# hahnyuan/PTQ4ViT

Hardware: AMD Instinct MI355X
Metric: calibration throughput (wrapped modules calibrated per second), ViT-B/224 W8A8, 32 calibration images (higher is better)
Workload: dtype int8

## Files before the change

ptq4vit_amd/csrc/p4v_api.hip:

```cpp
#include <hip/hip_runtime.h>

#include <algorithm>
#include <atomic>
#include <climits>
#include <cstdarg>
#include <cstdio>
#include <condition_variable>
#include <cstring>
#include <deque>
#include <functional>
#include <thread>
#include <mutex>
#include <string>
#include <unordered_map>
#include <type_traits>
#include <vector>

#include "../../include/ptq4vit_hip.h"
#include "../../include/ptq4vit_hip_debug.h"
#include "p4v_kernels.h"

using namespace p4v;

namespace {
// ... 499 lines not shown
    return p.mode == PACK_SYM && !p.conv && !(p.blk_mode == 1 && p.blk_div2) && p.lo >= -128 && p.hi <= 127 && p.lo <= p.hi &&
           (p.crange ? live_max == 1 : p.C == 1) && (p.c_inner != 3 || (p.Rp % 64 == 0 && p.Kp % 64 == 0));
}
std::atomic<int> g_pack_general{0};
template <typename T> int launch_pack(Ctx& c, const PackParams& p_, int live_max = -1) {
    if (c.dry) return 0;
    PackParams p = p_;
    if (p.crange && live_max == 0) return 0;
    p.qbias = (sizeof(T) == 1 && p.mode == PACK_SYM && p.lo == -128 && p.hi == 127 && tune(TUNE_B1_PATH) != 11) ? cvt_bias(c) : 0.0f;
    const long total = (long)p.Z * p.Rp * (p.Kp / 16);
    if (total >= (1L << 31)) return fail(P4V_ERR_UNSUPPORTED, "operand plane too large for k_pack (%ld 16-element runs)", total);
    const int groups = cdiv((p.crange && live_max > 0) ? std::min(p.C, live_max) : p.C, PACK_CG);
    const long cap = !p.crange ? 256L * 64 : live_max > 0 ? std::max(256L * 12, 256L * 64 / groups) : 256L * 12;
    const int blocks = (int)std::min<long>(cdiv(total, 256), cap);
    if (p.mode == PACK_TWIN_I8) {
        if (sizeof(T) != 1 || p.C != 1 || p.c_inner != 0 || !p.scales || p.conv || p.zdiv > 0)
            return fail(P4V_ERR_UNSUPPORTED, "merged twin plane: one fixed row-major int8 plane only");
        return enqueue(c, KERN(PackParams, k_pack_twin), dim3(blocks), dim3(256), 0, p);
    }
    const bool single = sizeof(T) == 1 && pack1_ok(p, live_max) && !g_pack_general.load(std::memory_order_relaxed);
    if (tune(TUNE_PRINT) > 1) fprintf(stderr, "[p4v] %s stage %d: Z %d Rp %d Kp %d C %d crange %d done %d live_max %d layout %d grid %d x %d\n", single ? "k_pack1" : "k_pack", g_stage, p.Z, p.Rp, p.Kp, p.C, p.crange != nullptr, p.done != nullptr, live_max, p.c_inner, blocks, single ? 1 : groups);
    if (single) return enqueue(c, KERN(PackParams, k_pack1), dim3(blocks), dim3(256), 0, p);
    return enqueue(c, KERN_T(PackParams, k_pack, T), dim3(blocks, groups), dim3(256), 0, p);
}

inline int lockstep(const Ctx& c, int kind) {
    if (!c.grp) return 1;
    const int seen = (kind >= 0 && kind < 16) ? c.grp->last_par[kind] : 0;
    return std::max(1, seen > 0 ? seen : c.par);
}
inline int cu_slots(const Ctx& c, int slots, int kind) { return std::max(8, slots / lockstep(c, kind)); }
#define P4V_EPI4(epi, X)                                   \
    switch (epi) {                                         \
        case EPI_SQ_W: { constexpr int E = EPI_SQ_W; X; }  \
        case EPI_SQ: { constexpr int E = EPI_SQ; X; }      \
        case EPI_ABS: { constexpr int E = EPI_ABS; X; }    \
        default: { constexpr int E = EPI_W_SQ; X; }        \
    }

template <typename T, bool TWIN> int launch_sweep_epi(Ctx& c, const SweepParams& p, int epi, int cgroups, const StatInfo* si) {
    const size_t lds = 2 * (TWIN ? 3 : 2) * SW_TILE_BYTES;
    dim3 grid(p.mtiles * p.ntiles, p.Z, cgroups), block(512);
    switch (epi) {
        case EPI_SQ_W: return enqueue(c, KERN_T(SweepParams, k_sweep, T, TWIN, EPI_SQ_W), grid, block, lds, p, si);
        case EPI_SQ: return enqueue(c, KERN_T(SweepParams, k_sweep, T, TWIN, EPI_SQ), grid, block, lds, p, si);
        case EPI_ABS: return enqueue(c, KERN_T(SweepParams, k_sweep, T, TWIN, EPI_ABS), grid, block, lds, p, si);
        case EPI_W_SQ: return enqueue(c, KERN_T(SweepParams, k_sweep, T, TWIN, EPI_W_SQ), grid, block, lds, p, si);
        case EPI_STORE: return enqueue(c, KERN1_T(SweepParams, k_sweep, T, TWIN, EPI_STORE), grid, block, lds, p, si);
        case EPI_FWD: return enqueue(c, KERN1_T(SweepParams, k_sweep, T, TWIN, EPI_FWD), grid, block, lds, p, si);
        default: return enqueue(c, KERN1_T(SweepParams, k_sweep, T, TWIN, EPI_COS), grid, block, lds, p, si);
    }
}

template <bool TWIN> int launch_sweep2g_epi(Ctx& c, const SweepParams& p, int epi, int cgroups, const StatInfo* si) {
    const int per = 2 * cdiv(p.c1 - p.c0, 2 * cgroups);
    const size_t lds = (size_t)SW2_NS * (TWIN ? 4 : 3) * SW2_TILE + (size_t)per * 8 * sizeof(float) * (TWIN ? 3 : 2);
    dim3 grid(p.mtiles * p.ntiles, p.Z, cgroups), block(512);
    P4V_EPI4(epi, return enqueue(c, KERN_T(SweepParams, k_sweep2g, TWIN, E), grid, block, lds, p, si))
}

template <bool TWIN> int launch_sweep2_epi(Ctx& c, const SweepParams& p, int epi, int cgroups, const StatInfo* si) {
    const int per = cdiv(p.c1 - p.c0, cgroups);
    const size_t lds = (size_t)SW2_NS * (TWIN ? 3 : 2) * SW2_TILE + (size_t)per * 8 * sizeof(float) * (TWIN ? 3 : 2);
    dim3 grid(p.mtiles * p.ntiles, p.Z, cgroups), block(512);
    switch (epi) {
        case EPI_SQ_W: return enqueue(c, KERN_T(SweepParams, k_sweep2, TWIN, EPI_SQ_W), grid, block, lds, p, si);
        case EPI_SQ: return enqueue(c, KERN_T(SweepParams, k_sweep2, TWIN, EPI_SQ), grid, block, lds, p, si);
        case EPI_ABS: return enqueue(c, KERN_T(SweepParams, k_sweep2, TWIN, EPI_ABS), grid, block, lds, p, si);
        case EPI_FWD: return enqueue(c, KERN1_T(SweepParams, k_sweep2, TWIN, EPI_FWD), grid, block, lds, p, si);
        case EPI_STORE:
            if constexpr (TWIN) return enqueue(c, KERN1_T(SweepParams, k_sweep2, TWIN, EPI_STORE), grid, block, lds, p, si);
            else return enqueue(c, KERN_T(SweepParams, k_sweep2, TWIN, EPI_STORE), grid, block, lds, p, si);
        case EPI_COS: return enqueue(c, KERN_T(SweepParams, k_sweep2, TWIN, EPI_COS), grid, block, lds, p, si);
        default: return enqueue(c, KERN_T(SweepParams, k_sweep2, TWIN, EPI_W_SQ), grid, block, lds, p, si);
    }
}

#ifdef P4V_TRACE
unsigned long long* g_trace = nullptr;
int trace_attach(Sweep3Params& p) {
    if (!g_trace) HIPCHK(hipMalloc(&g_trace, sizeof(unsigned long long) * 16 * 65536));
    p.trace = g_trace;
    return 0;
}
int trace_dump(Ctx& c, dim3 grid, int ktiles) {
    if (!getenv("P4V_TRACE_FILE")) return 0;
    const size_t n = (size_t)grid.x * grid.z * 16;
    HIPCHK(hipStreamSynchronize(c.st));
    std::vector<unsigned long long> h(n);
    HIPCHK(hipMemcpy(h.data(), g_trace, n * 8, hipMemcpyDeviceToHost));
    FILE* f = fopen(getenv("P4V_TRACE_FILE"), "ab");
    unsigned long long hdr[4] = {0xABCDull, grid.x, grid.z, (unsigned long long)ktiles};
    fwrite(hdr, 8, 4, f); fwrite(h.data(), 8, n, f); fclose(f);
    return 0;
}
#endif

inline StatInfo stat_info(int kind, double macs, double alg, int gx, int gz, double bytes) {
    return StatInfo{kind, macs * g_exec_frac, alg * g_exec_frac, g_stage, gx, gz, bytes};
}

enum SweepKind { SK_BOUND, SK_SWEEP6, SK_SWEEP5, SK_SWEEP7, SK_SWEEP7_TWIN, SK_SWEEP7_MERGED, SK_SWEEP9, SK_SWEEP8, SK_SWEEP2G, SK_SWEEP2,
                 SK_GENERIC_I8, SK_GENERIC_F32, SK_COUNT };
constexpr int SWEEP_RECORD_KIND[SK_COUNT] = {12, 2, 5, 3, 4, 4, 6, 7, 8, 9, 0, 1};
inline bool sweep_stationary(SweepKind k) { return k == SK_SWEEP6 || k == SK_SWEEP5; }
inline bool sweep_large_k(SweepKind k) { return k == SK_SWEEP7 || k == SK_SWEEP7_TWIN || k == SK_SWEEP7_MERGED; }

int launch_sweep5(Ctx& c, const Sweep3Params& p, int epi, int cgroups) {
    if (c.dry) return 0;
    const int per = 2 * cdiv(p.c1 - p.c0, 2 * cgroups);
    const size_t lds = (size_t)p.ktiles * SW2_TILE + (size_t)SW5_NP * 2 * SW2_TILE + (size_t)per * 8 * sizeof(float) * 2 + 256;
    dim3 grid(p.stiles * p.ttiles, 1, cgroups), block(512);
#ifdef P4V_TRACE
    CHK(trace_attach(const_cast<Sweep3Params&>(p)));
#endif
    const StatInfo si = stat_info(SWEEP_RECORD_KIND[SK_SWEEP5], (double)p.stiles * 128 * (double)p.ttiles * 128 * (double)p.ldk * (p.c1 - p.c0), g_alg_macs_cand * (p.c1 - p.c0),
                                  (int)grid.x, (int)grid.z, g_alg_bytes);
    const StatInfo* sp = &si;
    P4V_EPI4(epi, CHK(enqueue(c, KERN_T(Sweep3Params, k_sweep5, E), grid, block, lds, p, sp)); break)
#ifdef P4V_TRACE
    CHK(trace_dump(c, grid, p.ktiles));
#endif
    return 0;
}

template <int KT>
int launch_sweep6_kt(Ctx& c, const Sweep3Params& p, int epi, dim3 grid, size_t lds, const StatInfo* si) {
    if (epi == EPI_COS) return enqueue(c, KERN_T(Sweep3Params, k_sweep6, EPI_COS, KT, 2), grid, dim3(256), lds, p, si);
    if (epi == EPI_COS_T) return enqueue(c, KERN_T(Sweep3Params, k_sweep6, EPI_COS_T, KT, 2), grid, dim3(256), lds, p, si);
    P4V_EPI4(epi, return enqueue(c, KERN_T(Sweep3Params, k_sweep6, E, KT, 2), grid, dim3(256), lds, p, si))
}

bool sweep6_supported(int ktiles) { return ktiles == 3 || ktiles == 4 || ktiles == 6 || ktiles == 8 || ktiles == 12; }

int launch_sweep6_part(Ctx& c, const Sweep3Params& p, int epi, int cgroups);

int launch_sweep6(Ctx& c, const Sweep3Params& p, int epi, int cgroups, int nc_model = 0) {
    if (c.dry) return 0;
    const int tiles = p.ntile > 0 ? p.ntile : p.stiles * p.ttiles, base = p.ntile > 0 ? p.tile0 : 0;
    const int nc = nc_model > 0 ? nc_model : p.c1 - p.c0;
    const int full = tiles / 256 * 256, rem = tiles - full;
    const double P = tune(TUNE_P6) > 0 ? 0.1 * tune(TUNE_P6) : 20.0, t_c = 0.196 * p.ktiles;
    auto waves = [](long wgs) { return (double)((wgs + 255) / 256); };
    int q_best = 0;
    if (rem > 0 && full > 0 && lockstep(c, 2) <= 1) {
        double best = waves((long)tiles * cgroups) * (P + cdiv(nc, cgroups) * t_c) * 0.97;
        for (int q = 1; q <= std::min(nc, 12); ++q) {
            const double t = waves(full) * (P + nc * t_c) + waves((long)rem * q) * (P + cdiv(nc, q) * t_c);
            if (t < best) { best = t; q_best = q; }
        }
    }
    if (tune(TUNE_PRINT) > 0) fprintf(stderr, "[p4v] sweep6 tiles %d: full %d rem %d -> q %d (uniform cg %d)\n", tiles, full, rem, q_best, cgroups);
    if (q_best > 0) {
        Sweep3Params a = p, b = p;
        a.tile0 = base; a.ntile = full;
        b.tile0 = base + full; b.ntile = rem;
        CHK(launch_sweep6_part(c, a, epi, 1));
// ... 21 lines not shown
    int r;
    switch (p.ktiles) {
        case 12: r = launch_sweep6_kt<12>(c, p, epi, grid, lds, sp); break;
        case 8: r = launch_sweep6_kt<8>(c, p, epi, grid, lds, sp); break;
        case 6: r = launch_sweep6_kt<6>(c, p, epi, grid, lds, sp); break;
        case 4: r = launch_sweep6_kt<4>(c, p, epi, grid, lds, sp); break;
        default: r = launch_sweep6_kt<3>(c, p, epi, grid, lds, sp); break;
    }
    if (r) return r;
#ifdef P4V_TRACE
    CHK(trace_dump(c, grid, p.ktiles));
#endif
    return 0;
}

template <bool ROWS_FIXED> int launch_sweep9_epi(Ctx& c, const SweepParams& p, int epi, int cgroups, const StatInfo* si) {
    const int per = cdiv(p.c1 - p.c0, cgroups);
    const size_t lds = (size_t)SW9_NS * SW9_STAGE + (size_t)per * SW9_NW * sizeof(float) * 2;
    dim3 grid(p.halves, p.Z, cgroups), block(SW9_NW * 64);
    P4V_EPI4(epi, return enqueue(c, KERN_T(SweepParams, k_sweep9, ROWS_FIXED, E), grid, block, lds, p, si))
}

template <bool ROWS_FIXED> int launch_sweep8_epi(Ctx& c, const SweepParams& p, int epi, int cgroups, const StatInfo* si) {
    const int per = cdiv(p.c1 - p.c0, cgroups);
    const size_t lds = (size_t)SW8_NS * SW2_TILE + (size_t)per * 8 * sizeof(float) * 2;
    dim3 grid(p.mtiles * p.ntiles, p.Z, cgroups), block(512);
    P4V_EPI4(epi, return enqueue(c, KERN_T(SweepParams, k_sweep8, ROWS_FIXED, E, false), grid, block, lds, p, si))
}

template <int TWIN> int launch_sweep7_epi(Ctx& c, const Sweep7Params& p, int epi, dim3 grid, size_t lds, const StatInfo* si) {
    if constexpr (TWIN == 0) { if (epi == EPI_COS) return enqueue(c, KERN_T(Sweep7Params, k_sweep7, 0, EPI_COS), grid, dim3(512), lds, p, si); }
    if (epi == EPI_COS) return fail(P4V_ERR_UNSUPPORTED, "k_sweep7: the cosine epilogue has no twin instance");
    P4V_EPI4(epi, return enqueue(c, KERN_T(Sweep7Params, k_sweep7, TWIN, E), grid, dim3(512), lds, p, si))
}

int launch_sweep7(Ctx& c, const Sweep7Params& p, int twin, int epi, int cgroups) {
    if (c.dry) return 0;
    const int nc = p.c1 - p.c0;
    const int per_max = (int)((160 * 1024 - SW7_NS * SW7_STAGE - 256) / 192);
    cgroups = std::max(cgroups, cdiv(nc, per_max));
    const int per = cdiv(nc, cgroups);
    const size_t lds = (size_t)SW7_NS * SW7_STAGE + (size_t)per * 192 + 256;
    Sweep7Params q = p;
    q.cgroups = cgroups;
    dim3 grid(p.rtiles * p.ctiles * cgroups, 1, 1);
    const StatInfo si = stat_info(SWEEP_RECORD_KIND[twin ? SK_SWEEP7_TWIN : SK_SWEEP7], (double)p.rtiles * 256 * (double)p.ctiles * 256 * (double)p.ldk * nc, g_alg_macs_cand * nc,
                                  (int)grid.x, (int)grid.z, g_alg_bytes);
    const StatInfo* sp = &si;
    return twin == 2 ? launch_sweep7_epi<2>(c, q, epi, grid, lds, sp) : twin ? launch_sweep7_epi<1>(c, q, epi, grid, lds, sp) : launch_sweep7_epi<0>(c, q, epi, grid, lds, sp);
}

int launch_sweep(Ctx& c, const SweepParams& p, SweepKind kind, bool twin, int epi, int cgroups) {
    if (c.dry) return 0;
    const double kelems = (double)p.ldk / (kind == SK_GENERIC_F32 ? 4 : 1);
    const int tiles = p.mtiles * p.ntiles;
    auto record = [&](int gx) {
        return stat_info(SWEEP_RECORD_KIND[kind], (double)p.mtiles * SW_BM * (double)p.ntiles * SW_BN * kelems * p.Z * (p.c1 - p.c0) * (twin ? 2 : 1),
                         g_alg_macs_cand * (p.c1 - p.c0), gx, cgroups, g_alg_bytes);
    };
    switch (kind) {
        case SK_BOUND: {
            const bool prev = b1_previous();
            const StatInfo si = record(tiles * (prev ? 2 : 1));
            const dim3 grid(tiles * (prev ? 2 : 1)), block(256);
            if (prev) P4V_EPI4(epi, return enqueue(c, KERN_T(SweepParams, k_bound, E, 1), grid, block, 0, p, &si))
            P4V_EPI4(epi, return enqueue(c, KERN_T(SweepParams, k_bound, E, 2), grid, block, 0, p, &si))
        }
        case SK_SWEEP9: {
            const StatInfo si = record(p.halves);
            return p.a_cs == 0 ? launch_sweep9_epi<true>(c, p, epi, cgroups, &si) : launch_sweep9_epi<false>(c, p, epi, cgroups, &si);
        }
        case SK_SWEEP8: {
            const StatInfo si = record(tiles);
            return p.a_cs == 0 ? launch_sweep8_epi<true>(c, p, epi, cgroups, &si) : launch_sweep8_epi<false>(c, p, epi, cgroups, &si);
        }
        case SK_SWEEP2G: {
            const StatInfo si = record(tiles);
            return twin ? launch_sweep2g_epi<true>(c, p, epi, cgroups, &si) : launch_sweep2g_epi<false>(c, p, epi, cgroups, &si);
        }
        case SK_SWEEP2: {
            const StatInfo si = record(tiles);
            return twin ? launch_sweep2_epi<true>(c, p, epi, cgroups, &si) : launch_sweep2_epi<false>(c, p, epi, cgroups, &si);
        }
        case SK_GENERIC_I8: {
            const StatInfo si = record(tiles);
            return twin ? launch_sweep_epi<int8_t, true>(c, p, epi, cgroups, &si) : launch_sweep_epi<int8_t, false>(c, p, epi, cgroups, &si);
        }
        case SK_GENERIC_F32: {
            const StatInfo si = record(tiles);
            return twin ? launch_sweep_epi<float, true>(c, p, epi, cgroups, &si) : launch_sweep_epi<float, false>(c, p, epi, cgroups, &si);
        }
        default: return fail(P4V_ERR_INVALID, "launch_sweep: family %d has a launcher of its own", (int)kind);
    }
}

int launch_finish(Ctx& c, const FinishParams& p) {
    return enqueue(c, KERN(FinishParams, k_finish), dim3(p.C, p.nj), dim3(256), 0, p);
}

int launch_finish_cos(Ctx& c, const FinishCosParams& p) {
    const int gy = p.j_mode == 3 ? cdiv(p.S, 256) : p.nj;
    return enqueue(c, KERN(FinishCosParams, k_finish_cos), dim3(p.C, gy), dim3(p.j_mode == 3 ? 256 : 1024), 0, p);
}

int launch_select(Ctx& c, const SelectParams& p_) {
    if (c.dry) return 0;
    SelectParams p = p_;
    attach_mirror(p);
    return enqueue(c, KERN(SelectParams, k_select), dim3(p.nj), dim3(128), 0, p);
}

struct PlaneCache {
    char* buf = nullptr;
    bool assigned = false, valid = false;
    unsigned char* done = nullptr;
};
struct SliceCache {
    bool assigned = false;
    int k = 0;
    int k_eff = 0;
    int* idx = nullptr; float* mass = nullptr;
    float* Os = nullptr; float* Gs = nullptr; float* Rs = nullptr;
    const void* idx_src = nullptr; int idx_wt = -1;
    const void* o_src = nullptr; const void* g_src = nullptr; const void* r_src = nullptr;
    float* frac = nullptr;
    PlaneCache aplane;
    bool loose = false;
    float frac_host = 1.0f;
};
typedef PlaneCache EpiCache;

struct Operand {
    PackParams pk;
    bool expanded;
    bool present;
};

struct SegPlan {
    SegTable seg; unsigned char ablk[SEG_MAX], bblk[SEG_MAX]; int Kseg;
    int batch, H, M, K, N;
    int nVA, nHA, nVB, nHB, crA, ccA, crB, ccB;
    const float* A; long a_st[4]; const float* B; long b_st[4];
    int Aq, Bq; bool sos;
// ... 204 lines not shown
    long part_cs;
    long p_zs, p_cs; int NpP;
    int s3_groups, cos6_Sp;
    int h9;
    long fin_zs; int fin_ld, fin_rows, fin_cols, fin_jdiv;
};

int sweep9_halves(const Pass& ps, int ktiles) {
    const int epi = ps.epi;
    if (ktiles != 1 || ps.twin || ps.row.expanded == ps.col.expanded || epi == EPI_STORE || epi == EPI_FWD || epi == EPI_COS) return 0;
    if (ps.sb_mode == 1 && ps.s_cs > 1) return 0;
    if (ps.bias_axis != 0 || (g_variant & 524288)) return 0;
    if ((ps.row.expanded ? ps.Mrows : ps.Ncols) > 256) return 0;
    const long nb = (long)cdiv(ps.Mrows, 16) * cdiv(ps.Ncols, 16);
    const int halves = (int)cdiv(nb, (long)SW9_NW * SW9_NB);
    if (halves > 32 / SW9_NW) return 0;
    const double waste = (double)rup(ps.Mrows, 128) * rup(ps.Ncols, 128) / ((double)rup(ps.Mrows, 16) * rup(ps.Ncols, 16));
    return (waste >= 1.4 || (g_variant & 1048576)) ? halves : 0;
}
bool sweep8_ok(const Pass& ps, int ktiles) {
    return ktiles == 1 && !ps.twin && ps.row.expanded != ps.col.expanded && ps.epi != EPI_STORE && ps.epi != EPI_FWD && ps.epi != EPI_COS &&
           !(g_variant & 65536);
}
bool sweep2g_ok(const Pass& ps, int ktiles) {
    return ps.col.expanded && !ps.row.expanded && ktiles >= 16 && ps.o_bs == 0 && ps.o_nbs == 0 && ps.epi != EPI_COS;
}

int plan_sweep(const Ctx& c, const Pass& ps, SweepPlan& pl) {
    pl = SweepPlan{};
    const int esz = pl.esz = ps.i8 ? 1 : 4;
    const int Kp = pl.Kp = (int)rup(ps.K, 64 / esz);
    const int ktiles = Kp * esz / SW_BKB;
    const long K64 = rup(ps.K, 64);
    const bool cosm = ps.epi == EPI_COS, i8v2 = ps.i8 && !g_force_v1;
    const bool one_expanded = ps.row.expanded != ps.col.expanded, plain_out = ps.o_bs == 0 && ps.o_nbs == 0;
    const bool scale32 = ps.sb_mode != 1 || ps.s_cs == 1 || ps.sb_div % 32 == 0;
    const bool score32 = ps.j_mode == 0 || (ps.j_mode == 1 && (ps.nj == 1 || ps.j_div % 32 == 0));
    const bool blocks64 = (ps.s_cs == 1 || ps.sb_div % 64 == 0) && (ps.j_mode == 0 || (ps.j_mode == 1 && (ps.nj == 1 || ps.j_div % 64 == 0)));
    const bool bound = ps.bound_kernel && i8v2 && !ps.twin && ps.Z == 1 && !ps.store_out && !cosm && plain_out && ps.bias_axis == 0 &&
                       (ps.sb_mode == 0 || ps.sb_mode == 1) && score32 && scale32 && (ps.eq_n == 1 || ps.crange);
    const bool stat_ok = !bound && !ps.store_out && i8v2 && !ps.twin && (!cosm || ps.cos6) && !(g_variant & 4) && ps.Z == 1 &&
                         ps.sb_mode == 1 && blocks64 && one_expanded && K64 <= 768 && plain_out;
    const bool regs6 = stat_ok && sweep6_supported(ktiles);
    if (ps.cos6 && !regs6) return fail(P4V_ERR_UNSUPPORTED, "cosine pass planned for k_sweep6 does not qualify for it");
    const bool big7 = !bound && !stat_ok && !ps.store_out && i8v2 && (!cosm || ps.cos7) && !(g_variant & 32768) && ps.Z == 1 &&
                      K64 >= 1024 && K64 % 256 == 0 && (long)ps.Mrows * ps.o_ms * 4 < (1L << 32) && ps.sb_mode == 1 && scale32 && score32 &&
                      one_expanded && !(ps.twin && (ps.row.expanded || ps.row2.expanded)) &&
                      plain_out && ps.o_ns == 1 && ps.Ncols % 32 == 0 && ps.o_ms % 4 == 0 &&
                      (c.dry || ((((unsigned long long)ps.O) | ((unsigned long long)(ps.G ? ps.G : ps.O))) & 15) == 0) && ps.bias_axis == 0;
    if (ps.cos7 && (!big7 || ps.twin)) return fail(P4V_ERR_UNSUPPORTED, "cosine pass planned for k_sweep7 does not qualify for it");
    const bool fast = !stat_ok && i8v2 && !cosm && scale32 && (score32 || ps.j_mode == 2);
    pl.fast_cos = cosm && !stat_ok && !big7 && i8v2 && !ps.store_out && tune(TUNE_B1_PATH) != 7 && scale32;
    pl.pairs = stat_ok && !regs6;
    pl.merged7 = big7 && ps.twin && ps.twin_disjoint && !(g_variant & 2097152);
    pl.kind = bound ? SK_BOUND : regs6 ? SK_SWEEP6 : stat_ok ? SK_SWEEP5 :
              big7 ? (pl.merged7 ? SK_SWEEP7_MERGED : ps.twin ? SK_SWEEP7_TWIN : SK_SWEEP7) :
              !(fast || pl.fast_cos) ? (ps.i8 ? SK_GENERIC_I8 : SK_GENERIC_F32) :
              (fast && sweep8_ok(ps, ktiles)) ? SK_SWEEP8 : (fast && sweep2g_ok(ps, ktiles)) ? SK_SWEEP2G : SK_SWEEP2;
    const bool blk_ranges = ps.crange && ps.crange_blk && tune(TUNE_B1_PATH) != 9;
    pl.rblk = (blk_ranges && regs6 && !ps.row.expanded && ps.j_mode == 1 && ps.nj == ps.s_cs && ps.j_div == ps.sb_div) ? ps.crange_blk : nullptr;
    pl.rblk_z = (blk_ranges && !stat_ok && ps.j_mode == 2 && ps.nj == ps.j_div && ps.Z > 1 && !cosm && !ps.store_out && !bound && K64 < 1024)
                    ? ps.crange_blk : nullptr;
    const int Mp = pl.Mp = (int)rup(ps.Mrows, big7 ? (ps.twin ? 128 : 256) : (regs6 && !ps.row.expanded) ? 256 : SW_BM);
    const int Np = pl.Np = (int)rup(ps.Ncols, big7 ? 256 : (regs6 && !ps.col.expanded) ? 256 : SW_BM);
    pl.b64 = fast && !big7 && !bound && ps.Z > 1 && !ps.col_zs_shared && ps.Ncols <= 64 && ktiles >= 2 && ktiles <= 15 && !ps.store_out;
    pl.NpB = pl.b64 ? 64 : Np;
    pl.row_plane1 = (long)(ps.row_zs_shared ? 1 : ps.Z) * Mp * Kp * esz;
    pl.col_plane1 = (long)(ps.col_zs_shared ? 1 : ps.Z) * pl.NpB * Kp * esz;
    pl.exp_plane = ps.row.expanded ? pl.row_plane1 : pl.col_plane1;
    pl.chunk = (int)std::max<long>(1, std::min<long>(ps.eq_n, PLANE_BUDGET / std::max<long>(1, pl.exp_plane)));
    if (pl.pairs && pl.chunk > 1) pl.chunk &= ~1;
    pl.chunk_al = pl.pairs ? ((pl.chunk + 1) & ~1) : pl.chunk;
    pl.slack = stat_ok ? 4096 : 0;
    pl.cin_exp = bound ? 3 : stat_ok ? (pl.pairs ? 2 : 1) : 0;
    pl.cin_fix = (bound || regs6) ? 3 : 0;
    pl.zero_bias_n = stat_ok ? (size_t)std::max(Mp, Np) : 0;
    pl.epi7_n = big7 ? (size_t)Mp * Np * 2 : 0;
    const bool a_search = pl.a_search = ps.row.expanded;
    pl.s6_stiles = (a_search ? Np : Mp) / 256; pl.s6_ttiles = (int)cdiv(a_search ? ps.Mrows : ps.Ncols, 64);
    pl.epi6_on = regs6 && (a_search || ps.cos6 || tune(TUNE_EPI6W) == 1);
    pl.epi6_bytes = pl.epi6_on ? (size_t)pl.s6_stiles * pl.s6_ttiles * (256 * 64 * 8) : 0;
    const int MT = Mp / 64, s3_slabs = (a_search ? Np : Mp) / 64, s3_groups = pl.s3_groups = (a_search ? Mp : Np) / 32;
    const int NpP = pl.NpP = stat_ok ? s3_groups : fast ? Np / 32 : Np;
    const int MT7 = big7 ? (Mp / (ps.twin ? 128 : 256)) * 4 : 0;
    const bool cosp = ps.cos6 || ps.cos7;
    const int cos_slab = ps.cos7 ? 128 : 64;
    const int cos6_Sp = pl.cos6_Sp = ps.cos7 ? Mp : ps.cos6 ? (a_search ? (int)cdiv(ps.Mrows, 64) * 64 : Mp) : 0;
    const int cos6_slabs = ps.cos7 ? Np / 128 : ps.cos6 ? (a_search ? Np / 64 : (int)cdiv(ps.Ncols, 64)) : 0;
    pl.p_zs = cosp ? (long)cos6_slabs * cos6_Sp * 3 : stat_ok ? (long)s3_slabs * s3_groups : big7 ? (long)MT7 * NpP : (long)MT * NpP * (cosm ? 3 : 1);
    pl.p_cs = pl.part_cs = pl.p_zs * ps.Z;
    if (fast && !bound && !big7 && !ps.store_out && (ps.j_mode == 0 || ps.j_mode == 2)) {
        const int h9 = sweep9_halves(ps, ktiles);
        if (h9 > 0 && (long)h9 * SW9_NW <= pl.p_zs) { pl.kind = SK_SWEEP9; pl.h9 = h9; pl.p_zs = (long)h9 * SW9_NW; pl.p_cs = pl.p_zs * ps.Z; }
    }
    pl.fin_zs = pl.p_zs;
    if (pl.kind == SK_SWEEP9) {
        pl.fin_ld = pl.fin_cols = (int)pl.p_zs; pl.fin_rows = 1; pl.fin_jdiv = std::max(1, ps.j_div);
    } else if (!cosm) {
        pl.fin_ld = NpP; pl.fin_rows = stat_ok ? s3_slabs : big7 ? MT7 : MT;
        pl.fin_cols = stat_ok ? (a_search ? (regs6 ? 2 * cdiv(ps.Mrows, 64) : s3_groups) : cdiv(ps.Ncols, 32)) : fast ? cdiv(ps.Ncols, 32) : ps.Ncols;
        pl.fin_jdiv = std::max(1, (fast || stat_ok) && ps.j_mode == 1 ? cdiv(ps.j_div, 32) : ps.j_div);
    } else {
        const int FS = !cosp ? 0 : ps.cos_ZV == 1 ? cos6_slabs : ps.sb_div / cos_slab;
        if (cosp) pl.fin_zs = (long)FS * cos6_Sp * 3;
        pl.fin_ld = cosp ? cos6_Sp : Np; pl.fin_rows = cosp ? FS : MT; pl.fin_cols = cosp ? ps.Mrows : ps.Ncols;
        pl.fin_jdiv = std::max(1, ps.cos_j_div);
    }
    return 0;
}
inline SweepKind chunk_kind(const SweepPlan& pl, int nc) { return (pl.kind == SK_SWEEP2G && nc < 2) ? SK_SWEEP2 : pl.kind; }
// ... 195 lines not shown
    q.r_cs = ps.col.expanded ? pl.col_plane1 : 0;
    q.R = b.col - (long)c0 * q.r_cs;
    q.c_cs = ps.row.expanded ? pl.row_plane1 : 0;
    q.Cp = b.row - (long)c0 * q.c_cs;
    q.C2 = pl.kind == SK_SWEEP7_TWIN ? b.row2 : nullptr;
    q.ldk = pl.Kp; q.ktiles = pl.Kp / SW_BKB;
    q.S1 = b.S1; q.S2 = b.S2; q.s_cs = ps.s_cs; q.sb_div = ps.s_cs > 1 ? std::max(1, ps.sb_div) : (1 << 30);
    q.E = b.epi7;
    q.c0 = c0; q.c1 = c0 + nc; q.crange = ps.crange;
    q.part = b.part; q.p_cs = pl.p_cs; q.NG = ps.cos7 ? pl.cos6_Sp : pl.NpP;
    q.rtiles = pl.Np / 256; q.ctiles = pl.Mp / (ps.twin ? 128 : 256);
    int cg7 = choose_cgroups((long)q.rtiles * q.ctiles, nc, q.ktiles + 3, cu_slots(c, 256, SWEEP_RECORD_KIND[ps.twin ? SK_SWEEP7_TWIN : SK_SWEEP7]), 6.0, 0.62, 100);
    if (tune(TUNE_CG7) > 0) cg7 = std::max(1, std::min(nc, tune(TUNE_CG7)));
    q.order = tune(TUNE_ORDER7) > 0 ? tune(TUNE_ORDER7) - 1 : 1;
    if (tune(TUNE_PRINT) > 0) fprintf(stderr, "[p4v] sweep7 tiles %d x %d ktiles %d cand %d twin %d -> cgroups %d\n", q.rtiles, q.ctiles, q.ktiles, nc, (int)ps.twin, cg7);
    if (pl.kind == SK_SWEEP7_MERGED) { q.twin_s = ps.row.pk.scales; q.C2 = b.row2; }
    return launch_sweep7(c, q, pl.kind == SK_SWEEP7_MERGED ? 2 : ps.twin ? 1 : 0, ps.epi, cg7);
}

int sweep_chunk_tiled(Ctx& c, const Pass& ps, const SweepPlan& pl, const PassBufs& b, SweepKind kind, int c0, int nc) {
    const int esz = pl.esz, Mp = pl.Mp, Np = pl.Np, Kp = pl.Kp;
    SweepParams sp{};
    sp.a_cs = ps.row.expanded ? pl.row_plane1 : 0;
    sp.A = b.row - (long)c0 * sp.a_cs;
    sp.a_zs = ps.row_zs_shared ? 0 : (long)Mp * Kp * esz;
    if (ps.twin) {
        sp.a2_cs = ps.row2.expanded ? pl.row_plane1 : 0;
        sp.A2 = b.row2 - (long)c0 * sp.a2_cs;
        sp.a2_zs = sp.a_zs;
    }
    sp.b_cs = ps.col.expanded ? pl.col_plane1 : 0;
    sp.B = b.col - (long)c0 * sp.b_cs;
    sp.b_zs = ps.col_zs_shared ? 0 : (long)pl.NpB * Kp * esz;
    sp.b_rows = pl.b64 ? 64 : 0;
    sp.ldk = Kp * esz; sp.ktiles = sp.ldk / SW_BKB;
    sp.S1 = b.S1; sp.S2 = b.S2; sp.s_cs = ps.s_cs; sp.sb_mode = ps.sb_mode; sp.sb_div = std::max(1, ps.sb_div);
    sp.bias = ps.bias; sp.bias_axis = ps.bias_axis; sp.bias_zs = ps.bias_zs;
    sp.O = ps.O; sp.Wt = ps.G ? ps.G : ps.O; sp.wt_mode = ps.wt_mode;
    sp.o_zs = ps.o_zs; sp.o_bs = ps.o_bs; sp.o_ms = ps.o_ms; sp.o_nbs = ps.o_nbs; sp.o_ns = ps.o_ns;
    sp.o_inner = ps.o_inner > 0 ? ps.o_inner : INT_MAX;
    sp.o_ninner = ps.o_ninner > 0 ? ps.o_ninner : INT_MAX;
    sp.M = ps.Mrows; sp.N = ps.Ncols; sp.Z = ps.Z; sp.c0 = c0; sp.c1 = c0 + nc; sp.crange = ps.crange;
    sp.crange_blk = pl.rblk_z; sp.cb_div = std::max(1, ps.j_div);
    sp.part = b.part; sp.p_cs = pl.p_cs; sp.p_zs = pl.p_zs; sp.Np = pl.NpP;
    sp.mtiles = Mp / SW_BM; sp.ntiles = Np / SW_BN;
    sp.dbg = g_variant & 3;
    sp.store = ps.store_out;
    const long wgs = (long)sp.mtiles * sp.ntiles * ps.Z;
    int cgroups;
    switch (kind) {
        case SK_GENERIC_I8: case SK_GENERIC_F32:
            cgroups = choose_cgroups(wgs, nc, sp.ktiles, cu_slots(c, 512, SWEEP_RECORD_KIND[kind]), 20.0, ps.i8 ? 1.6 : 2.6);
            break;
        case SK_SWEEP9:
            sp.halves = pl.h9;
            sp.rows_p_stream = sp.a_cs == 0 ? Np : Mp;
            cgroups = choose_cgroups((long)pl.h9 * ps.Z, nc, 1, cu_slots(c, SW9_NW == 4 ? 512 : 256, SWEEP_RECORD_KIND[SK_SWEEP9]), 12.0, 0.9);
            break;
        case SK_BOUND:
            sp.bound = 1;
            sp.dbg = tune(TUNE_B1_PATH) >= 16 ? (tune(TUNE_B1_PATH) >> 4) : 0;
            sp.A = b.row; sp.B = b.col; sp.a_cs = sp.b_cs = 0;
            [[fallthrough]];
        default:
            cgroups = choose_cgroups(wgs, nc, sp.ktiles, cu_slots(c, ps.twin ? 256 : 512, SWEEP_RECORD_KIND[SK_SWEEP2]), ps.twin ? 40.0 : 25.0, ps.twin ? 0.45 : 0.40);
    }
    const bool tuned = kind != SK_GENERIC_I8 && kind != SK_GENERIC_F32 && !pl.fast_cos && !ps.store_out;
    if (tuned) {
        const char* g = kind == SK_SWEEP2G ? "g" : "";
        if (const int t_ = tune(kind == SK_SWEEP2G ? TUNE_CG2G : TUNE_CG2); t_ > 0) cgroups = std::max(1, std::min(nc, t_));
        if (tune(TUNE_PRINT) > 0) fprintf(stderr, "[p4v] sweep2%s tiles %d x %d z %d ktiles %d cand %d twin %d -> cgroups %d\n", g, sp.mtiles, sp.ntiles, ps.Z, sp.ktiles, nc, (int)ps.twin, cgroups);
    }
    return launch_sweep(c, sp, kind, ps.twin, ps.epi, cgroups);
}

int finish_pass(Ctx& c, const Pass& ps, const SweepPlan& pl, const PassBufs& b) {
    if (ps.epi == EPI_COS) {
        FinishCosParams fp{b.part, pl.p_cs, pl.fin_zs, pl.fin_ld, pl.fin_rows, ps.cos_ZB, ps.cos_ZV, pl.fin_cols, ps.eq_n,
                           ps.cos_j_mode, pl.fin_jdiv, ps.nj, ps.norm, b.scores};
        return launch_finish_cos(c, fp);
    }
    FinishParams fp{b.part, pl.p_cs, pl.fin_zs, pl.fin_ld, pl.fin_rows, ps.Z, pl.fin_cols, ps.eq_n, ps.j_mode, pl.fin_jdiv, ps.nj, ps.norm,
                    b.scores, ps.crange};
    if (ps.crange && b.pc && b.pc->done) { fp.mark_done = b.pc->done; fp.mark_n = ps.eq_n; }
    fp.crange_blk = pl.rblk ? pl.rblk : pl.rblk_z;
    return launch_finish(c, fp);
}

int run_pass(Ctx& c, Pass& ps) {
    if (ps.seg) return run_pass_seg(c, ps);
    g_alg_macs_cand = (double)ps.Mrows * ps.Ncols * ps.K * ps.Z;
    g_alg_bytes = 4.0 * ((double)ps.Mrows * ps.K * (ps.row_zs_shared ? 1 : ps.Z) + (double)ps.Ncols * ps.K * (ps.col_zs_shared ? 1 : ps.Z)) +
                  (ps.G ? 8.0 : 4.0) * (double)ps.Mrows * ps.Ncols * ps.Z;
    SweepPlan pl;
    CHK(plan_sweep(c, ps, pl));
    const size_t mark = c.ws.off;
    PassBufs b{};
    CHK(pass_workspace(c, ps, pl, b));
    if (ps.pack_only) {
        if (b.pc && ps.row.expanded != ps.col.expanded && !ps.crange) CHK(pack_expanded(c, ps, pl, b, 0, ps.eq_n));
        c.ws.off = mark;
        return 0;
    }
    CHK(prep_epilogue(c, ps, pl, b));
    if (ps.use_s1 && !ps.s_ready) {
        ps.s1.S = b.S1; ps.s1.C = ps.eq_n; ps.s1.nblk = ps.s_cs;
        CHK(launch_scale(c, ps.s1));
        if (ps.twin) { ps.s2.S = b.S2; ps.s2.C = ps.eq_n; ps.s2.nblk = ps.s_cs; CHK(launch_scale(c, ps.s2)); }
    }
    CHK(pack_fixed_planes(c, ps, pl, b));
    for (int c0 = 0; c0 < ps.eq_n; c0 += pl.chunk) {
        const int nc = std::min(pl.chunk, ps.eq_n - c0);
        CHK(pack_expanded(c, ps, pl, b, c0, nc));
        CHK(chunk_exec_frac(c, ps, pl, c0, nc));
        const SweepKind kind = chunk_kind(pl, nc);
        if (sweep_stationary(kind)) CHK(sweep_chunk_stationary(c, ps, pl, b, c0, nc));
        else if (sweep_large_k(kind)) CHK(sweep_chunk_large_k(c, ps, pl, b, c0, nc));
        else CHK(sweep_chunk_tiled(c, ps, pl, b, kind, c0, nc));
    }
    g_exec_frac = 1.0;
// ... 2328 lines not shown
```

ptq4vit_amd/csrc/p4v_kernels.h:

```cpp
#pragma once
#include <hip/hip_runtime.h>
#include <stdint.h>
#include <type_traits>

namespace p4v {

typedef int v4i __attribute__((ext_vector_type(4)));
typedef int v16i __attribute__((ext_vector_type(16)));
typedef float v4f __attribute__((ext_vector_type(4)));
typedef float v16f __attribute__((ext_vector_type(16)));
typedef float v2f __attribute__((ext_vector_type(2)));

#ifndef P4V_GROUP_KERNARG
#define P4V_GROUP_KERNARG (4096 - 256)
#endif
template <typename P> struct GroupArgs {
    static constexpr int CAP_RAW = (P4V_GROUP_KERNARG - 16) / (int)(sizeof(P) + 16);
    static constexpr int CAP = CAP_RAW > 64 ? 64 : CAP_RAW;
    int n;
    unsigned off[CAP + 1];
    unsigned gx[CAP], gy[CAP], gz[CAP];
    P p[CAP];
};
#define P4V_BIDX uint3{blockIdx.x, blockIdx.y, blockIdx.z}
// ... 1153 lines not shown
                    float* q = p.part + (long)c * p.p_cs + (long)z * p.p_zs + ((long)(mt * 2 + wr) * p.Np + n0 + wc * 32 + l31) * 3;
                    q[0] = dot; q[1] = nn; q[2] = oo;
                }
                kt = 0;
                ++c;
                return;
            }
            v2f sum2 = {0.0f, 0.0f};
#pragma unroll
            for (int i = 0; i < 2; ++i) {
                if (i == 1 && !act1) break;
#pragma unroll
                for (int r = 0; r < 16; r += 2) {
                    const v2f a = {(float)acc[i][r], (float)acc[i][r + 1]};
                    const v2f uu = {u[i][r], u[i][r + 1]};
                    const v2f ww = {w[i][r], w[i][r + 1]};
                    v2f d = uu - a * s1;
                    if (TWIN) { const v2f a2 = {(float)acc2[i][r], (float)acc2[i][r + 1]}; d = d - a2 * s2; }
                    if (EPI == EPI_SQ_W) { const v2f t2 = ww * d; sum2 = t2 * t2 + sum2; }
                    else if (EPI == EPI_SQ) sum2 = d * d + sum2;
                    else if (EPI == EPI_ABS) sum2 += v2f{fabsf(d.x), fabsf(d.y)};
                    else sum2 = (ww * d) * d + sum2;
                    acc[i][r] = 0; acc[i][r + 1] = 0;
                    if (TWIN) { acc2[i][r] = 0; acc2[i][r + 1] = 0; }
                }
            }
            const float sum = wave_sum_dpp(sum2.x + sum2.y);
            if (lane == 63) res[(c - c_lo) * 8 + pos] = sum;
            kt = 0;
            ++c;
        }
    };
    if (total > 2) wait_vmcnt<NPL * 2>(); else if (total > 1) wait_vmcnt<NPL>(); else wait_vmcnt<0>();
    __builtin_amdgcn_s_barrier();
    read_fr(fa, std::integral_constant<int, 0>{});
    for (int it = 0; it < total; it += SW2_NS) {
        tile(it, std::integral_constant<int, 0>{}, fa, fb);
        if (it + 1 < total) tile(it + 1, std::integral_constant<int, 1>{}, fb, fa);
        if (it + 2 < total) tile(it + 2, std::integral_constant<int, 2>{}, fa, fb);
        if (it + 3 < total) tile(it + 3, std::integral_constant<int, 3>{}, fb, fa);
    }
#undef P4V_DSR
    __syncthreads();
    if constexpr (STORES || EPI == EPI_COS) return;
    for (int i = tid; i < (c_hi - c_lo) * 8; i += 512) {
        const int cc = c_lo + i / 8, wv = i % 8;
        p.part[(long)cc * p.p_cs + (long)z * p.p_zs + (long)(mt * 2 + (wv >> 2)) * p.Np + nt * 4 + (wv & 3)] = res[i];
    }
}
template <bool TWIN, int EPI>
__global__ __launch_bounds__(512, 2) void k_sweep2(SweepParams p) { k_sweep2_body<TWIN, EPI>(p, P4V_BIDX, P4V_GDIM); }
template <bool TWIN, int EPI>
__global__ __launch_bounds__(512, 2) void k_sweep2_g(GroupArgs<SweepParams> a) { P4V_GROUP_ENTER(a); k_sweep2_body<TWIN, EPI>(a.p[m_], vb_, vg_); }

template <int EPI, int NB>
__device__ __forceinline__ void k_bound_body(const SweepParams& p, const uint3 blockIdx, const uint3 gridDim) {
    static_assert(NB == 1 || NB == 2, "k_bound: one or two 32-column blocks per wave");
    const int tid = threadIdx.x, lane = tid & 63;
    const int wid = __builtin_amdgcn_readfirstlane(tid >> 6);
    const int g = lane >> 5, l31 = lane & 31;
    const int ntiles = p.ntiles * (2 / NB);
    const int nwg = p.mtiles * ntiles;
    const int t = xcd_remap(blockIdx.x, nwg);
    constexpr int GM = 4;
    const int per_group = GM * ntiles;
    const int first_m = (t / per_group) * GM;
    const int gsz = min(p.mtiles - first_m, GM);
    const int mt = first_m + (t % per_group) % gsz, nt = (t % per_group) / gsz;
    int c = p.c0;
    if (p.crange) {
        const int a = __builtin_amdgcn_readfirstlane(p.crange[0]), b = __builtin_amdgcn_readfirstlane(p.crange[1]);
        if (a >= b) return;
        c = max(c, a);
        if (c >= b) return;
    }
    if (c >= p.c1) return;
    const int wr = wid >> 1, wc = wid & 1;
    const int m0 = mt * 128 + wr * 64, n0 = nt * (64 * NB) + wc * (32 * NB);
    float* slot = p.part + (long)c * p.p_cs + (long)(mt * 2 + wr) * p.Np + (n0 >> 5);
    if (m0 >= p.M || n0 >= p.N) {
        if (lane == 63) {
#pragma unroll
            for (int j = 0; j < NB; ++j) slot[j] = 0.0f;
        }
        return;
    }
    const char* sA = (const char*)p.A + (long)(m0 >> 6) * p.ktiles * 4096;
    const char* sB = (const char*)p.B + (long)(n0 >> 6) * p.ktiles * 4096 + (NB == 1 ? ((n0 >> 5) & 1) * 2048 : 0);
    const unsigned vo = (unsigned)lane * 16u;
    v16i acc[2][NB];
#pragma unroll
    for (int i = 0; i < 2; ++i)
#pragma unroll
        for (int j = 0; j < NB; ++j)
#pragma unroll
            for (int r = 0; r < 16; ++r) acc[i][j][r] = 0;
    struct Fr { v4i a[2][2], b[NB][2]; };
#define P4V_BLD(dst, voff, sbase, off) asm volatile("global_load_dwordx4 %0, %1, %2 offset:%3" : "=v"(dst) : "v"(voff), "s"(sbase), "n"(off) : "memory")
    auto load = [&](Fr& f) __attribute__((always_inline)) {
        P4V_BLD(f.a[0][0], vo, sA, 0); P4V_BLD(f.a[0][1], vo, sA, 1024);
        P4V_BLD(f.b[0][0], vo, sB, 0); P4V_BLD(f.b[0][1], vo, sB, 1024);
        P4V_BLD(f.a[1][0], vo, sA, 2048); P4V_BLD(f.a[1][1], vo, sA, 3072);
        if constexpr (NB == 2) { P4V_BLD(f.b[1][0], vo, sB, 2048); P4V_BLD(f.b[1][1], vo, sB, 3072); }
        sA += 4096; sB += 4096;
    };
    auto mma = [&](Fr& f) __attribute__((always_inline)) {
// ... 2970 lines not shown
```

Before: 680.5.

## Add pipelined fp32 MFMA sweep kernel for non-int8 difference-epilogue candidate passes

Adds k_sweepf, a dedicated fp32 candidate-sweep kernel. It keeps an 8-slot LDS ring fed by async global-to-LDS loads, double-buffers fragment reads, runs 32x32x2 f32 MFMAs, and folds the squared, abs or weighted-difference epilogue in registers per candidate. Reference outputs, weights and per-candidate scales are preloaded once into registers and an LDS table. Non-int8, non-twin, non-store passes that previously used the generic fp32 sweep are routed to it, with their own cgroup selection capped by the LDS scale table size. The aim is to cut the memory stalls and epilogue overhead of the generic float path, at the cost of LDS capacity limits and another code path to maintain.

```diff
diff --git a/ptq4vit_amd/csrc/p4v_api.hip b/ptq4vit_amd/csrc/p4v_api.hip
--- a/ptq4vit_amd/csrc/p4v_api.hip
+++ b/ptq4vit_amd/csrc/p4v_api.hip
@@ -575,6 +575,14 @@
     }
 }
 
+int launch_sweepf_epi(Ctx& c, const SweepParams& p, int epi, int cgroups, const StatInfo* si) {
+    const int per = cdiv(p.c1 - p.c0, cgroups);
+    if (per > SWF_PER_MAX) return fail(P4V_ERR_INVALID, "k_sweepf: %d candidates per workgroup exceed the scale table (%d)", per, SWF_PER_MAX);
+    const size_t lds = (size_t)SWF_RING + (size_t)per * SWF_CAND_BYTES;
+    dim3 grid(p.mtiles * p.ntiles, p.Z, cgroups), block(512);
+    P4V_EPI4(epi, return enqueue(c, KERN_T(SweepParams, k_sweepf, E), grid, block, lds, p, si))
+}
+
 template <bool TWIN> int launch_sweep2g_epi(Ctx& c, const SweepParams& p, int epi, int cgroups, const StatInfo* si) {
     const int per = 2 * cdiv(p.c1 - p.c0, 2 * cgroups);
     const size_t lds = (size_t)SW2_NS * (TWIN ? 4 : 3) * SW2_TILE + (size_t)per * 8 * sizeof(float) * (TWIN ? 3 : 2);
@@ -624,8 +632,8 @@
 }
 
 enum SweepKind { SK_BOUND, SK_SWEEP6, SK_SWEEP5, SK_SWEEP7, SK_SWEEP7_TWIN, SK_SWEEP7_MERGED, SK_SWEEP9, SK_SWEEP8, SK_SWEEP2G, SK_SWEEP2,
-                 SK_GENERIC_I8, SK_GENERIC_F32, SK_COUNT };
-constexpr int SWEEP_RECORD_KIND[SK_COUNT] = {12, 2, 5, 3, 4, 4, 6, 7, 8, 9, 0, 1};
+                 SK_GENERIC_I8, SK_GENERIC_F32, SK_PIPE_F32, SK_COUNT };
+constexpr int SWEEP_RECORD_KIND[SK_COUNT] = {12, 2, 5, 3, 4, 4, 6, 7, 8, 9, 0, 1, 1};
 inline bool sweep_stationary(SweepKind k) { return k == SK_SWEEP6 || k == SK_SWEEP5; }
 inline bool sweep_large_k(SweepKind k) { return k == SK_SWEEP7 || k == SK_SWEEP7_TWIN || k == SK_SWEEP7_MERGED; }
 
@@ -753,7 +761,7 @@
 
 int launch_sweep(Ctx& c, const SweepParams& p, SweepKind kind, bool twin, int epi, int cgroups) {
     if (c.dry) return 0;
-    const double kelems = (double)p.ldk / (kind == SK_GENERIC_F32 ? 4 : 1);
+    const double kelems = (double)p.ldk / ((kind == SK_GENERIC_F32 || kind == SK_PIPE_F32) ? 4 : 1);
     const int tiles = p.mtiles * p.ntiles;
     auto record = [&](int gx) {
         return stat_info(SWEEP_RECORD_KIND[kind], (double)p.mtiles * SW_BM * (double)p.ntiles * SW_BN * kelems * p.Z * (p.c1 - p.c0) * (twin ? 2 : 1),
@@ -790,6 +798,10 @@
         case SK_GENERIC_F32: {
             const StatInfo si = record(tiles);
             return twin ? launch_sweep_epi<float, true>(c, p, epi, cgroups, &si) : launch_sweep_epi<float, false>(c, p, epi, cgroups, &si);
+        }
+        case SK_PIPE_F32: {
+            const StatInfo si = record(tiles);
+            return launch_sweepf_epi(c, p, epi, cgroups, &si);
         }
         default: return fail(P4V_ERR_INVALID, "launch_sweep: family %d has a launcher of its own", (int)kind);
     }
@@ -1100,10 +1112,12 @@
     const bool fast = !stat_ok && i8v2 && !cosm && scale32 && (score32 || ps.j_mode == 2);
     pl.fast_cos = cosm && !stat_ok && !big7 && i8v2 && !ps.store_out && tune(TUNE_B1_PATH) != 7 && scale32;
     pl.pairs = stat_ok && !regs6;
+    const bool pipe_f32 = !ps.i8 && !ps.twin && !ps.store_out && (g_variant & 3) == 0 && tune(TUNE_B1_PATH) != 17 &&
+                          (ps.epi == EPI_SQ_W || ps.epi == EPI_SQ || ps.epi == EPI_ABS || ps.epi == EPI_W_SQ);
     pl.merged7 = big7 && ps.twin && ps.twin_disjoint && !(g_variant & 2097152);
     pl.kind = bound ? SK_BOUND : regs6 ? SK_SWEEP6 : stat_ok ? SK_SWEEP5 :
               big7 ? (pl.merged7 ? SK_SWEEP7_MERGED : ps.twin ? SK_SWEEP7_TWIN : SK_SWEEP7) :
-              !(fast || pl.fast_cos) ? (ps.i8 ? SK_GENERIC_I8 : SK_GENERIC_F32) :
+              !(fast || pl.fast_cos) ? (ps.i8 ? SK_GENERIC_I8 : pipe_f32 ? SK_PIPE_F32 : SK_GENERIC_F32) :
               (fast && sweep8_ok(ps, ktiles)) ? SK_SWEEP8 : (fast && sweep2g_ok(ps, ktiles)) ? SK_SWEEP2G : SK_SWEEP2;
     const bool blk_ranges = ps.crange && ps.crange_blk && tune(TUNE_B1_PATH) != 9;
     pl.rblk = (blk_ranges && regs6 && !ps.row.expanded && ps.j_mode == 1 && ps.nj == ps.s_cs && ps.j_div == ps.sb_div) ? ps.crange_blk : nullptr;
@@ -1405,6 +1419,11 @@
         case SK_GENERIC_I8: case SK_GENERIC_F32:
             cgroups = choose_cgroups(wgs, nc, sp.ktiles, cu_slots(c, 512, SWEEP_RECORD_KIND[kind]), 20.0, ps.i8 ? 1.6 : 2.6);
             break;
+        case SK_PIPE_F32:
+            cgroups = choose_cgroups(wgs, nc, sp.ktiles, cu_slots(c, 256, SWEEP_RECORD_KIND[kind]), 8.0, 1.2);
+            if (const int t_ = tune(TUNE_CG2); t_ > 0) cgroups = std::max(1, std::min(nc, t_));
+            cgroups = std::max(cgroups, cdiv(nc, SWF_PER_MAX));
+            break;
         case SK_SWEEP9:
             sp.halves = pl.h9;
             sp.rows_p_stream = sp.a_cs == 0 ? Np : Mp;
@@ -1412,13 +1431,13 @@
             break;
         case SK_BOUND:
             sp.bound = 1;
-            sp.dbg = tune(TUNE_B1_PATH) >= 16 ? (tune(TUNE_B1_PATH) >> 4) : 0;
+            sp.dbg = (tune(TUNE_B1_PATH) == 16 || tune(TUNE_B1_PATH) == 32) ? (tune(TUNE_B1_PATH) >> 4) : 0;
             sp.A = b.row; sp.B = b.col; sp.a_cs = sp.b_cs = 0;
             [[fallthrough]];
         default:
             cgroups = choose_cgroups(wgs, nc, sp.ktiles, cu_slots(c, ps.twin ? 256 : 512, SWEEP_RECORD_KIND[SK_SWEEP2]), ps.twin ? 40.0 : 25.0, ps.twin ? 0.45 : 0.40);
     }
-    const bool tuned = kind != SK_GENERIC_I8 && kind != SK_GENERIC_F32 && !pl.fast_cos && !ps.store_out;
+    const bool tuned = kind != SK_GENERIC_I8 && kind != SK_GENERIC_F32 && kind != SK_PIPE_F32 && !pl.fast_cos && !ps.store_out;
     if (tuned) {
         const char* g = kind == SK_SWEEP2G ? "g" : "";
         if (const int t_ = tune(kind == SK_SWEEP2G ? TUNE_CG2G : TUNE_CG2); t_ > 0) cgroups = std::max(1, std::min(nc, t_));
diff --git a/ptq4vit_amd/csrc/p4v_kernels.h b/ptq4vit_amd/csrc/p4v_kernels.h
--- a/ptq4vit_amd/csrc/p4v_kernels.h
+++ b/ptq4vit_amd/csrc/p4v_kernels.h
@@ -1229,6 +1229,221 @@
 __global__ __launch_bounds__(512, 2) void k_sweep2(SweepParams p) { k_sweep2_body<TWIN, EPI>(p, P4V_BIDX, P4V_GDIM); }
 template <bool TWIN, int EPI>
 __global__ __launch_bounds__(512, 2) void k_sweep2_g(GroupArgs<SweepParams> a) { P4V_GROUP_ENTER(a); k_sweep2_body<TWIN, EPI>(a.p[m_], vb_, vg_); }
+
+static constexpr int SWF_KS = 2, SWF_NS = 4, SWF_SLOTS = SWF_KS * SWF_NS;
+static constexpr int SWF_SLOT = 2 * SW2_TILE;
+static constexpr int SWF_RING = SWF_SLOTS * SWF_SLOT;
+static constexpr int SWF_CAND_BYTES = SW_BN * (int)sizeof(float);
+static constexpr int SWF_PER_MAX = (160 * 1024 - SWF_RING) / SWF_CAND_BYTES;
+
+template <int EPI>
+__device__ __forceinline__ void k_sweepf_body(const SweepParams& p, const uint3 blockIdx, const uint3 gridDim) {
+    static_assert(EPI == EPI_SQ_W || EPI == EPI_SQ || EPI == EPI_ABS || EPI == EPI_W_SQ, "k_sweepf: difference epilogues only");
+    extern __shared__ __attribute__((aligned(16))) char smem[];
+    float* s1tab = reinterpret_cast<float*>(smem + SWF_RING);
+
+    const int tid = threadIdx.x, lane = tid & 63;
+    const int wid = __builtin_amdgcn_readfirstlane(tid >> 6);
+    const int wr = wid >> 2, wc = wid & 3;
+    const int g = lane >> 5, l31 = lane & 31;
+
+    const int nwg = p.mtiles * p.ntiles;
+    const int t = xcd_remap(blockIdx.x, nwg);
+    const int mt = t % p.mtiles, nt = t / p.mtiles;
+    const int z = blockIdx.y, zc = blockIdx.z;
+    const int m0 = mt * SW_BM, n0 = nt * SW_BN;
+    const int per = (p.c1 - p.c0 + gridDim.z - 1) / gridDim.z;
+    int c_lo_ = p.c0 + zc * per, c_hi_ = min(p.c1, c_lo_ + per);
+    clip_crange(p.crange, c_lo_, c_hi_);
+    if (p.crange_blk) clip_crange_blk(p.crange_blk, z % p.cb_div, c_lo_, c_hi_);
+    const int c_lo = c_lo_, c_hi = c_hi_;
+    if (c_lo >= c_hi) return;
+
+    const int ld_row = wid * 16 + (lane >> 2);
+    const int ld_chunk = (lane & 3) ^ ((ld_row >> 2) & 3);
+    const unsigned voff = (unsigned)(ld_row * p.ldk + ld_chunk * 16);
+    const char* curA = (const char*)p.A + (long)z * p.a_zs + (long)m0 * p.ldk + (long)c_lo * p.a_cs;
+    const char* curB = (const char*)p.B + (long)z * p.b_zs + (long)n0 * p.ldk + (long)c_lo * p.b_cs;
+    const int ktiles = p.ktiles;
+    const long wrapA = p.a_cs - (long)ktiles * SW_BKB, wrapB = p.b_cs - (long)ktiles * SW_BKB;
+    const int lds_wave = wid * 1024;
+    const int total = (c_hi - c_lo) * ktiles;
+    int ikt = 0, iss = 0, islot = 0;
+    auto issue = [&]() __attribute__((always_inline)) {
+        if (iss >= total) return;
+        char* s = smem + islot * SWF_SLOT + lds_wave;
+        glds16(curA + voff, s);
+        glds16(curB + voff, s + SW2_TILE);
+        curA += SW_BKB; curB += SW_BKB;
+        if (++ikt == ktiles) { ikt = 0; curA += wrapA; curB += wrapB; }
+        islot = islot + 1 == SWF_SLOTS ? 0 : islot + 1;
+        ++iss;
+    };
+#pragma unroll
+    for (int i = 0; i < (SWF_NS - 1) * SWF_KS; ++i) issue();
+
+    float u[2][16], w[2][16];
+    const int n = n0 + wc * 32 + l31;
+    const bool ncol_ok = n < p.N;
+    const float bias_n = (p.bias && ncol_ok && p.bias_axis == 0) ? p.bias[(long)z * p.bias_zs + n] : 0.0f;
+    {
+        const int nc = min(n, p.N - 1);
+        const bool dense = p.o_inner == INT_MAX && p.o_ninner == INT_MAX;
+        const bool has_w = p.wt_mode == 1;
+        long idx[2][16];
+        if (dense) {
+            const long ncol_off = (long)z * p.o_zs + (long)nc * p.o_ns;
+#pragma unroll
+            for (int i = 0; i < 2; ++i)
+#pragma unroll
+                for (int r = 0; r < 16; ++r)
+                    idx[i][r] = ncol_off + (long)min(m0 + wr * 64 + i * 32 + (r & 3) + 8 * (r >> 2) + 4 * g, p.M - 1) * p.o_ms;
+        } else {
+            const long ncol_off = (long)z * p.o_zs + (long)(nc / p.o_ninner) * p.o_nbs + (long)(nc % p.o_ninner) * p.o_ns;
+#pragma unroll
+            for (int i = 0; i < 2; ++i)
+#pragma unroll
+                for (int r = 0; r < 16; ++r) {
+                    const int mc = min(m0 + wr * 64 + i * 32 + (r & 3) + 8 * (r >> 2) + 4 * g, p.M - 1);
+                    idx[i][r] = ncol_off + (long)(mc / p.o_inner) * p.o_bs + (long)(mc % p.o_inner) * p.o_ms;
+                }
+        }
+#pragma unroll
+        for (int i = 0; i < 2; ++i)
+#pragma unroll
+            for (int r = 0; r < 16; ++r) u[i][r] = p.O[idx[i][r]];
+        if (has_w) {
+#pragma unroll
+            for (int i = 0; i < 2; ++i)
+#pragma unroll
+                for (int r = 0; r < 16; ++r) w[i][r] = p.Wt[idx[i][r]];
+        } else {
+#pragma unroll
+            for (int i = 0; i < 2; ++i)
+#pragma unroll
+                for (int r = 0; r < 16; ++r) w[i][r] = 0.0f;
+        }
+        for (int i = tid; i < (c_hi - c_lo) * SW_BN; i += 512) {
+            const int col = n0 + (i & (SW_BN - 1));
+            const int sb = p.sb_mode == 1 ? min(col / p.sb_div, p.s_cs - 1) : p.sb_mode == 2 ? z % p.sb_div : 0;
+            s1tab[i] = p.S1 ? p.S1[(c_lo + (i >> 7)) * p.s_cs + sb] : 1.0f;
+        }
+        auto finish_uw = [&](auto wm_c) __attribute__((always_inline)) {
+            constexpr int WM = decltype(wm_c)::value;
+#pragma unroll
+            for (int i = 0; i < 2; ++i)
+#pragma unroll
+                for (int r = 0; r < 16; ++r) {
+                    const int m = m0 + wr * 64 + i * 32 + (r & 3) + 8 * (r >> 2) + 4 * g;
+                    const bool ok = ncol_ok && m < p.M;
+                    const float o = u[i][r], gw = w[i][r];
+                    const float ov = o - bias_n;
+                    const float wv = WM == 1 ? gw : WM == 2 ? o : WM == 3 ? fabsf(o) : 1.0f;
+                    u[i][r] = ok ? ov : 0.0f;
+                    w[i][r] = ok ? wv : 0.0f;
+                }
+        };
+        switch (p.wt_mode) {
+            case 1: finish_uw(std::integral_constant<int, 1>{}); break;
+            case 2: finish_uw(std::integral_constant<int, 2>{}); break;
+            case 3: finish_uw(std::integral_constant<int, 3>{}); break;
+            default: finish_uw(std::integral_constant<int, 0>{}); break;
+        }
+    }
+    __syncthreads();
+
+    v16f acc[2];
+#pragma unroll
+    for (int i = 0; i < 2; ++i)
+#pragma unroll
+        for (int r = 0; r < 16; ++r) acc[i][r] = 0.0f;
+
+    const int ra = wr * 64 + l31, rb = wc * 32 + l31;
+    const int sa = (ra >> 2) & 3, sbz = (rb >> 2) & 3;
+    const unsigned lds0 = (unsigned)(unsigned long long)(__attribute__((address_space(3))) char*)smem;
+    const unsigned aA0 = lds0 + ra * 64 + (((2 * g) ^ sa) << 4), aA1 = lds0 + ra * 64 + (((2 * g + 1) ^ sa) << 4);
+    const unsigned aB0 = lds0 + SW2_TILE + rb * 64 + (((2 * g) ^ sbz) << 4), aB1 = lds0 + SW2_TILE + rb * 64 + (((2 * g + 1) ^ sbz) << 4);
+
+#define P4V_DSRF(dst, addr, off) asm volatile("ds_read_b128 %0, %1 offset:%2" : "=v"(dst) : "v"(addr), "n"(off))
+    struct Fr { v4f b0, b1, a00, a01, a10, a11; };
+    auto read_fr = [&](Fr& f, int slot) __attribute__((always_inline)) {
+        const unsigned so = (unsigned)(slot * SWF_SLOT);
+        const unsigned xA0 = aA0 + so, xA1 = aA1 + so, xB0 = aB0 + so, xB1 = aB1 + so;
+        P4V_DSRF(f.b0, xB0, 0); P4V_DSRF(f.a00, xA0, 0); P4V_DSRF(f.a10, xA0, 2048);
+        P4V_DSRF(f.b1, xB1, 0); P4V_DSRF(f.a01, xA1, 0); P4V_DSRF(f.a11, xA1, 2048);
+    };
+    int kt = 0, c = c_lo;
+    auto tile = [&](Fr& f) __attribute__((always_inline)) {
+        asm volatile("" : "+v"(f.b0), "+v"(f.b1), "+v"(f.a00), "+v"(f.a01), "+v"(f.a10), "+v"(f.a11) :: "memory");
+#pragma unroll
+        for (int e = 0; e < 4; ++e) {
+            acc[0] = __builtin_amdgcn_mfma_f32_32x32x2f32(f.a00[e], f.b0[e], acc[0], 0, 0, 0);
+            acc[1] = __builtin_amdgcn_mfma_f32_32x32x2f32(f.a10[e], f.b0[e], acc[1], 0, 0, 0);
+        }
+#pragma unroll
+        for (int e = 0; e < 4; ++e) {
+            acc[0] = __builtin_amdgcn_mfma_f32_32x32x2f32(f.a01[e], f.b1[e], acc[0], 0, 0, 0);
+            acc[1] = __builtin_amdgcn_mfma_f32_32x32x2f32(f.a11[e], f.b1[e], acc[1], 0, 0, 0);
+        }
+        if (++kt == ktiles) {
+            const float s1 = s1tab[(c - c_lo) * SW_BN + wc * 32 + l31];
+            float colsum = 0.0f;
+#pragma unroll
+            for (int i = 0; i < 2; ++i)
+#pragma unroll
+                for (int r = 0; r < 16; ++r) {
+                    const float o_sim = acc[i][r] * s1;
+                    const float d = u[i][r] - o_sim;
+                    if (EPI == EPI_SQ_W) { const float tt = w[i][r] * d; colsum = fmaf(tt, tt, colsum); }
+                    else if (EPI == EPI_SQ) colsum = fmaf(d, d, colsum);
+                    else if (EPI == EPI_ABS) colsum += fabsf(d);
+                    else colsum = fmaf(w[i][r] * d, d, colsum);
+                    acc[i][r] = 0.0f;
+                }
+            colsum += __shfl_xor(colsum, 32);
+            if (g == 0) p.part[(long)c * p.p_cs + (long)z * p.p_zs + (long)(mt * 2 + wr) * p.Np + n0 + wc * 32 + l31] = colsum;
+            kt = 0;
+            ++c;
+        }
+    };
+
+    Fr fa, fb;
+    const int nst = (total + SWF_KS - 1) / SWF_KS;
+    int slot = 0;
+    read_fr(fa, 0);
+    for (int s = 0; s < nst; ++s) {
+        const int after = total - SWF_KS * (s + 2);
+        if (after >= 2) wait_vmcnt<4>(); else if (after == 1) wait_vmcnt<2>(); else wait_vmcnt<0>();
+        __builtin_amdgcn_s_barrier();
+        issue();
+        issue();
+        const bool two = total - SWF_KS * s >= 2;
+        const bool more = s + 1 < nst;
+        const int nslot = slot + SWF_KS == SWF_SLOTS ? 0 : slot + SWF_KS;
+        if (two) {
+            read_fr(fb, slot + 1);
+            __builtin_amdgcn_s_waitcnt(0xC07F | (6 << 8));
+        } else {
+            __builtin_amdgcn_s_waitcnt(0xC07F);
+        }
+        tile(fa);
+        if (two) {
+            if (more) {
+                read_fr(fa, nslot);
+                __builtin_amdgcn_s_waitcnt(0xC07F | (6 << 8));
+            } else {
+                __builtin_amdgcn_s_waitcnt(0xC07F);
+            }
+            tile(fb);
+        }
+        slot = nslot;
+    }
+#undef P4V_DSRF
+}
+template <int EPI>
+__global__ __launch_bounds__(512, 2) void k_sweepf(SweepParams p) { k_sweepf_body<EPI>(p, P4V_BIDX, P4V_GDIM); }
+template <int EPI>
+__global__ __launch_bounds__(512, 2) void k_sweepf_g(GroupArgs<SweepParams> a) { P4V_GROUP_ENTER(a); k_sweepf_body<EPI>(a.p[m_], vb_, vg_); }
 
 template <int EPI, int NB>
 __device__ __forceinline__ void k_bound_body(const SweepParams& p, const uint3 blockIdx, const uint3 gridDim) {
```

New measurement: 685.0 (median of 5 runs). No clear change (+0.7%).
